# Lucaskabela/UNAST

Hardware: AMD Instinct MI355X
Metric: mel-frames/sec/node (train step, gen+disc) at B=32,T_mel=800; 1/2/4/8-GPU scaling (higher is better)
Workload: dtype bf16x3

## Files before the change

unast_amd/csrc/loss.hip:

```cpp
#include "common.h"

__global__ __launch_bounds__(256) void speech_loss_fwd_kernel(const float* __restrict__ gold, const float* __restrict__ head, int ldh,
                                                              const float* __restrict__ post, const int* __restrict__ lens, int B, int T, int M,
                                                              float eos_weight, double* __restrict__ ws, float* __restrict__ loss) {
    const int rows = B * T;
    const int mq = M >> 2;
    const size_t total = (size_t)rows * mq;
    float a0 = 0.f, a1 = 0.f, a2 = 0.f;
    for (size_t i = (size_t)blockIdx.x * 256 + threadIdx.x; i < total; i += (size_t)gridDim.x * 256) {
        const int r = (int)(i / mq), c = (int)(i - (size_t)r * mq) * 4;
        const int b = r / T, t = r - b * T;
        const int len = lens[b];
        if (t < len) {
            float4 g = *reinterpret_cast<const float4*>(gold + (size_t)r * M + c);
            float4 p = *reinterpret_cast<const float4*>(head + (size_t)r * ldh + c);
            float4 q = *reinterpret_cast<const float4*>(post + (size_t)r * M + c);
            float d;
            d = g.x - p.x; a0 += d * d; d = g.y - p.y; a0 += d * d; d = g.z - p.z; a0 += d * d; d = g.w - p.w; a0 += d * d;
            d = g.x - q.x; a1 += d * d; d = g.y - q.y; a1 += d * d; d = g.z - q.z; a1 += d * d; d = g.w - q.w; a1 += d * d;
        }
        if (c == 0) {
            const float x = head[(size_t)r * ldh + M];
            const float y = (t == len - 1) ? 1.f : 0.f;
            const float lw = 1.f + (eos_weight - 1.f) * y;
// ... 189 lines not shown
                lg[c2][r] = v;
                if (n < V) mx = fmaxf(mx, v);
            }
        mx = fmaxf(mx, __shfl_xor(mx, 16, 64));
        mx = fmaxf(mx, __shfl_xor(mx, 32, 64));
        float se = 0.f, ly = 0.f;
#pragma unroll
        for (int c2 = 0; c2 < 3; ++c2)
#pragma unroll
            for (int r = 0; r < 4; ++r) {
                const int n = 16 * c2 + 4 * g + r;
                if (n < V) se += expf(lg[c2][r] - mx);
                if (n == y) ly = lg[c2][r];
            }
        se += __shfl_xor(se, 16, 64); se += __shfl_xor(se, 32, 64);
        ly += __shfl_xor(ly, 16, 64); ly += __shfl_xor(ly, 32, 64);
        const float wy = (y == pad_idx) ? 0.f : (y == eos_idx ? eos_weight : 1.f);
        const float inv = 1.f / se;
        if (mok) {
#pragma unroll
            for (int c2 = 0; c2 < 3; ++c2) {
                const int n0 = 16 * c2 + 4 * g;
                float4 lo4, dl4;
                float* lp = &lo4.x; float* dp = &dl4.x;
#pragma unroll
                for (int r = 0; r < 4; ++r) {
                    const int n = n0 + r;
                    lp[r] = n < V ? lg[c2][r] : 0.f;
                    dp[r] = n < V ? kg * wy * (expf(lg[c2][r] - mx) * inv - (n == y ? 1.f : 0.f)) : 0.f;
                }
                if (n0 < ldl) {
                    *reinterpret_cast<float4*>(logits + (size_t)m * ldl + n0) = lo4;
                    *reinterpret_cast<float4*>(dlogits + (size_t)m * ldl + n0) = dl4;
                }
            }
            if (g == 0) { a_nll = wy * (logf(se) + mx - ly); a_w = wy; }
        }
    }
    double da = wave_sum_d((double)a_nll), dw = wave_sum_d((double)a_w);
    if (lane == 0 && m0 < rows) { atomicAdd(ws + 0, da); atomicAdd(ws + 1, dw); }
    __syncthreads();
    if (t == 0) {
        __threadfence();
        const unsigned long long arrived = atomicAdd(reinterpret_cast<unsigned long long*>(ws + 3), 1ull) + 1ull;
        if (arrived == gridDim.x) {
            __threadfence();
            const double s0 = atomicAdd(ws + 0, 0.0), s1 = atomicAdd(ws + 1, 0.0);
            loss[0] = (float)(s0 / s1);
            ws[4] = s1;
            ws[0] = 0.0; ws[1] = 0.0; reinterpret_cast<unsigned long long*>(ws)[3] = 0ull;
        }
    }
}

__global__ __launch_bounds__(512) void speech_head_loss_kernel(const float* __restrict__ X, int ldx, const float* __restrict__ W, const float* __restrict__ bias,
                                                               const float* __restrict__ gold, const int* __restrict__ lens, int B, int T, int M,
                                                               float eos_weight, float gscale, float* __restrict__ head, float* __restrict__ d_head, int ldh,
                                                               double* __restrict__ ws) {
    extern __shared__ __attribute__((aligned(16))) unsigned char sdyn[];
    unsigned char* sw0 = sdyn;
    unsigned char* sw1 = sdyn + 96 * 512;
    __shared__ float s_denom;
    const int t = threadIdx.x, lane = t & 63, wave = t >> 6, l15 = lane & 15, g = lane >> 4;
    const int rows = B * T, NO = M + 1;
    for (int i = t; i < 96 * 64; i += 512) {
        const int n = i >> 6, c = (i & 63) * 4;
        float4 v = make_float4(0.f, 0.f, 0.f, 0.f);
        if (n < NO) v = *reinterpret_cast<const float4*>(W + (size_t)n * 256 + c);
        u32x2 hi, lo;
        split4<3>(v, hi, lo);
        *reinterpret_cast<u32x2*>(sw0 + whl_off(n, c)) = hi;
        *reinterpret_cast<u32x2*>(sw1 + whl_off(n, c)) = lo;
    }
    if (t == 0) {
        double sl = 0.0;
        for (int b = 0; b < B; ++b) sl += (double)lens[b];
        s_denom = (float)(sl * (double)M);
    }
    __syncthreads();
    const float km = 2.f * gscale / s_denom, ks = gscale / (float)rows;
    const int m0 = blockIdx.x * 128 + wave * 16;
    const int m = m0 + l15;
    const bool mok = m < rows;
    f32x4 acc[6];
#pragma unroll
    for (int c2 = 0; c2 < 6; ++c2) acc[c2] = (f32x4){0.f, 0.f, 0.f, 0.f};
    float a0 = 0.f, a2 = 0.f;
    if (m0 < rows) {
        const float* xr = X + (size_t)min(m, rows - 1) * ldx;
#pragma unroll
        for (int ks8 = 0; ks8 < 8; ++ks8) {
            const float4 a = *reinterpret_cast<const float4*>(xr + 32 * ks8 + 8 * g);
            const float4 c = *reinterpret_cast<const float4*>(xr + 32 * ks8 + 8 * g + 4);
            u32x2 h0, l0, h1, l1;
            split4<3>(a, h0, l0);
            split4<3>(c, h1, l1);
            const bf16x8_t xh = __builtin_bit_cast(bf16x8_t, (u32x4){h0[0], h0[1], h1[0], h1[1]});
            const bf16x8_t xl = __builtin_bit_cast(bf16x8_t, (u32x4){l0[0], l0[1], l1[0], l1[1]});
#pragma unroll
            for (int c2 = 0; c2 < 6; ++c2) {
                const int off = whl_off(16 * c2 + l15, 32 * ks8 + 8 * g);
                const bf16x8_t wh = *reinterpret_cast<const bf16x8_t*>(sw0 + off);
                const bf16x8_t wlo = *reinterpret_cast<const bf16x8_t*>(sw1 + off);
                acc[c2] = mfma16(wlo, xh, acc[c2]);
                acc[c2] = mfma16(wh, xl, acc[c2]);
                acc[c2] = mfma16(wh, xh, acc[c2]);
            }
        }
        if (mok) {
            const int b = m / T, tt = m - b * T;
            const int len = lens[b];
            const bool live = tt < len;
#pragma unroll
            for (int c2 = 0; c2 < 6; ++c2) {
                const int n0 = 16 * c2 + 4 * g;
                if (n0 >= ldh) continue;
                float4 hv = make_float4(0.f, 0.f, 0.f, 0.f), dv = hv;
                float* hp = &hv.x; float* dp = &dv.x;
                if (n0 < M) {
                    const float4 b4 = *reinterpret_cast<const float4*>(bias + n0);
                    const float bb[4] = {b4.x, b4.y, b4.z, b4.w};
                    float gd[4] = {0.f, 0.f, 0.f, 0.f};
                    if (live) { const float4 g4 = *reinterpret_cast<const float4*>(gold + (size_t)m * M + n0); gd[0] = g4.x; gd[1] = g4.y; gd[2] = g4.z; gd[3] = g4.w; }
#pragma unroll
                    for (int r = 0; r < 4; ++r) {
                        const float p = acc[c2][r] + bb[r];
                        hp[r] = p;
                        if (live) { const float d = p - gd[r]; a0 += d * d; dp[r] = km * d; }
                    }
                } else if (n0 == M) {
                    const float x = acc[c2][0] + bias[M];
                    const float y = (tt == len - 1) ? 1.f : 0.f;
                    const float lw = 1.f + (eos_weight - 1.f) * y;
                    hp[0] = x;
                    a2 += (1.f - y) * x + lw * (log1pf(expf(-fabsf(x))) + fmaxf(-x, 0.f));
                    dp[0] = ks * ((1.f - y) - lw * (1.f - 1.f / (1.f + expf(-x))));
                }
                *reinterpret_cast<float4*>(head + (size_t)m * ldh + n0) = hv;
                *reinterpret_cast<float4*>(d_head + (size_t)m * ldh + n0) = dv;
            }
        }
    }
    __shared__ double red[8][2];
    const double d0 = wave_sum_d((double)a0), d2 = wave_sum_d((double)a2);
    if (lane == 0) { red[wave][0] = d0; red[wave][1] = d2; }
    __syncthreads();
    if (t < 2) {
        double v = 0.0;
        for (int w = 0; w < 8; ++w) v += red[w][t];
        atomicAdd(ws + (t == 0 ? 0 : 2), v);
    }
}

__global__ __launch_bounds__(256) void speech_post_loss_kernel(const float* __restrict__ gold, const float* __restrict__ post, const int* __restrict__ lens,
                                                               int B, int T, int M, float gscale, float* __restrict__ d_post, double* __restrict__ ws,
                                                               float* __restrict__ loss) {
    __shared__ float s_denom;
    if (threadIdx.x == 0) {
        double sl = 0.0;
        for (int b = 0; b < B; ++b) sl += (double)lens[b];
        s_denom = (float)(sl * (double)M);
    }
    __syncthreads();
    const float km = 2.f * gscale / s_denom;
    const int rows = B * T, mq = M >> 2;
    const size_t total = (size_t)rows * mq;
    float a1 = 0.f;
    for (size_t i = (size_t)blockIdx.x * 256 + threadIdx.x; i < total; i += (size_t)gridDim.x * 256) {
        const int r = (int)(i / mq), c = (int)(i - (size_t)r * mq) * 4;
        const int b = r / T, t = r - b * T;
        float4 o = make_float4(0.f, 0.f, 0.f, 0.f);
        if (t < lens[b]) {
            const float4 g = *reinterpret_cast<const float4*>(gold + (size_t)r * M + c);
            const float4 q = *reinterpret_cast<const float4*>(post + (size_t)r * M + c);
            const float dx = q.x - g.x, dy = q.y - g.y, dz = q.z - g.z, dw = q.w - g.w;
            a1 += (dx * dx + dy * dy) + (dz * dz + dw * dw);
            o = make_float4(km * dx, km * dy, km * dz, km * dw);
        }
        *reinterpret_cast<float4*>(d_post + (size_t)r * M + c) = o;
    }
    __shared__ double red[4];
    const double d1 = wave_sum_d((double)a1);
    if ((threadIdx.x & 63) == 0) red[threadIdx.x >> 6] = d1;
    __syncthreads();
    if (threadIdx.x == 0) {
        atomicAdd(ws + 1, (red[0] + red[1]) + (red[2] + red[3]));
        __threadfence();
        const unsigned long long arrived = atomicAdd(reinterpret_cast<unsigned long long*>(ws + 3), 1ull) + 1ull;
        if (arrived == gridDim.x) {
            __threadfence();
            const double s0 = atomicAdd(ws + 0, 0.0), s1 = atomicAdd(ws + 1, 0.0), s2 = atomicAdd(ws + 2, 0.0);
            const double denom = (double)s_denom;
            loss[0] = (float)(s0 / denom + s1 / denom + s2 / ((double)B * T));
            ws[0] = 0.0; ws[1] = 0.0; ws[2] = 0.0; reinterpret_cast<unsigned long long*>(ws)[3] = 0ull;
        }
    }
}

__global__ __launch_bounds__(256) void disc_targets_kernel(const int64_t* __restrict__ perm, int n, int B, int flip, float smoothing, float* __restrict__ out) {
    for (int i = threadIdx.x; i < n; i += 256) {
        float y = 1.f - smoothing;
        if (perm[i] >= B) y = 1.f - y;
        if (flip) y = 1.f - y;
        out[i] = y;
    }
}

__global__ __launch_bounds__(256) void bce_logits_kernel(const float* __restrict__ logits, int ldx, const float* __restrict__ targets, int n,
                                                         const float* __restrict__ gscale, float* __restrict__ loss, float* __restrict__ dlogits, int ldd) {
    __shared__ float red[4];
    float a = 0.f;
    const float g = gscale ? gscale[0] : 0.f;
    for (int i = threadIdx.x; i < n; i += 256) {
        const float y = targets[i];
        const float x = logits[(size_t)i * ldx];
        a += (1.f - y) * x + log1pf(expf(-fabsf(x))) + fmaxf(-x, 0.f);
        if (dlogits) dlogits[(size_t)i * ldd] = g * (1.f / (1.f + expf(-x)) - y) / (float)n;
    }
    a = wave_sum(a);
    if ((threadIdx.x & 63) == 0) red[threadIdx.x >> 6] = a;
    __syncthreads();
    if (threadIdx.x == 0 && loss) loss[0] = ((red[0] + red[1]) + (red[2] + red[3])) / (float)n;
}

static int ls_grid(size_t work, int cap = 1024) {
    size_t b = (work + 255) / 256;
    if (b < 1) b = 1;
    if (b > (size_t)cap) b = cap;
    return (int)b;
}

extern "C" int unast_speech_loss_fwd(const float* gold, const float* head, int ldh, const float* post, const int* lens, int B, int T, int M,
                                     float eos_weight, double* ws , float* loss, hipStream_t stream) {
    UNAST_REQUIRE(gold && head && post && lens && ws && loss, "unast_speech_loss_fwd: null pointer");
    UNAST_REQUIRE(B > 0 && T > 0 && (M & 3) == 0 && ldh > M && (ldh & 3) == 0, "unast_speech_loss_fwd: need M%%4==0 and ldh>M, ldh%%4==0");
    hipLaunchKernelGGL(speech_loss_fwd_kernel, dim3(ls_grid((size_t)B * T * (M / 4), 512)), dim3(256), 0, stream, gold, head, ldh, post, lens, B, T, M,
                       eos_weight, ws, loss);
    return unast_check_launch("unast_speech_loss_fwd");
}

extern "C" int unast_speech_loss_bwd(const float* gold, const float* head, int ldh, const float* post, const int* lens, int B, int T, int M,
                                     float eos_weight, const float* gscale, float* d_head, float* d_post, hipStream_t stream) {
    UNAST_REQUIRE(gold && head && post && lens && gscale && d_head && d_post, "unast_speech_loss_bwd: null pointer");
    UNAST_REQUIRE(B > 0 && T > 0 && (M & 3) == 0 && ldh > M && (ldh & 3) == 0, "unast_speech_loss_bwd: need M%%4==0 and ldh>M, ldh%%4==0");
    hipLaunchKernelGGL(speech_loss_bwd_kernel, dim3(ls_grid((size_t)B * T * (ldh / 4))), dim3(256), 0, stream, gold, head, ldh, post, lens, B, T, M,
                       eos_weight, gscale, d_head, d_post);
    return unast_check_launch("unast_speech_loss_bwd");
}

extern "C" int unast_text_loss_fwd(const float* logits, int ldl, const int64_t* gold, int rows, int V, float eos_weight,
                                   double* ws , float* loss, hipStream_t stream) {
    UNAST_REQUIRE(logits && gold && ws && loss && rows > 0 && V > 0 && ldl >= V, "unast_text_loss_fwd: bad arguments");
    hipLaunchKernelGGL(text_loss_fwd_kernel, dim3(ls_grid(rows)), dim3(256), 0, stream, logits, ldl, gold, rows, V, 2, eos_weight, 0, ws, loss);
    return unast_check_launch("unast_text_loss_fwd");
}

extern "C" int unast_text_loss_bwd(const float* logits, int ldl, const int64_t* gold, int rows, int V, float eos_weight, const double* ws,
                                   const float* gscale, float* dlogits, hipStream_t stream) {
    UNAST_REQUIRE(logits && gold && ws && gscale && dlogits && rows > 0 && V > 0 && ldl >= V, "unast_text_loss_bwd: bad arguments");
    hipLaunchKernelGGL(text_loss_bwd_kernel, dim3(ls_grid(rows)), dim3(256), 0, stream, logits, ldl, gold, rows, V, 2, eos_weight, 0, ws, gscale, dlogits);
    return unast_check_launch("unast_text_loss_bwd");
}

__global__ __launch_bounds__(256) void randperm_kernel(long long* __restrict__ out, int n, uint32_t seed, uint32_t stream) {
    __shared__ uint32_t keys[4096];
    const uint32_t rk = rng_row_key(seed, stream, 0x9E3779B9u);
    for (int i = threadIdx.x; i < n; i += 256) keys[i] = rng_u32(rk, (uint32_t)i);
    __syncthreads();
    for (int i = threadIdx.x; i < n; i += 256) {
        const uint32_t k = keys[i];
        int r = 0;
        for (int j = 0; j < n; ++j) {
            const uint32_t kj = keys[j];
            r += (kj < k || (kj == k && j < i)) ? 1 : 0;
        }
        out[r] = i;
    }
}

extern "C" int unast_randperm(int64_t* out, int n, unsigned int seed, unsigned int stream_id, hipStream_t stream) {
    UNAST_REQUIRE(out && n > 0 && n <= 4096, "unast_randperm: need 0 < n <= 4096 (got %d)", n);
    hipLaunchKernelGGL(randperm_kernel, dim3(1), dim3(256), 0, stream, (long long*)out, n, seed, stream_id);
    return unast_check_launch("unast_randperm");
}

extern "C" int unast_disc_targets(const int64_t* perm, int n, int B, int flip, float smoothing, float* out, hipStream_t stream) {
    UNAST_REQUIRE(perm && out && n > 0, "unast_disc_targets: bad arguments");
    hipLaunchKernelGGL(disc_targets_kernel, dim3(1), dim3(256), 0, stream, perm, n, B, flip, smoothing, out);
    return unast_check_launch("unast_disc_targets");
}

extern "C" int unast_bce_logits(const float* logits, int ldx, const float* targets, int n, const float* gscale, float* loss, float* dlogits,
                                int ldd, hipStream_t stream) {
    UNAST_REQUIRE(logits && targets && n > 0 && ldx >= 1, "unast_bce_logits: bad arguments");
    UNAST_REQUIRE((dlogits == nullptr) || (gscale && ldd >= 1), "unast_bce_logits: dlogits requires gscale and ldd");
    hipLaunchKernelGGL(bce_logits_kernel, dim3(1), dim3(256), 0, stream, logits, ldx, targets, n, gscale, loss, dlogits, ldd);
    return unast_check_launch("unast_bce_logits");
}

__global__ __launch_bounds__(256) void masked_mse_kernel(const float* __restrict__ gold, const float* __restrict__ pred, const float* __restrict__ mask,
                                                         size_t n, double* __restrict__ ws, float* __restrict__ out) {
    double num = 0.0, den = 0.0;
    for (size_t i = (size_t)blockIdx.x * 256 + threadIdx.x; i < n; i += (size_t)gridDim.x * 256) {
        const float d = gold[i] - pred[i], m = mask[i];
        num += (double)(d * d * m);
        den += (double)m;
    }
    num = wave_sum_d(num);
    den = wave_sum_d(den);
    __shared__ double sn[4], sd[4];
    if ((threadIdx.x & 63) == 0) { sn[threadIdx.x >> 6] = num; sd[threadIdx.x >> 6] = den; }
    __syncthreads();
    if (threadIdx.x == 0) {
        atomicAdd(ws + 0, (sn[0] + sn[1]) + (sn[2] + sn[3]));
        atomicAdd(ws + 1, (sd[0] + sd[1]) + (sd[2] + sd[3]));
        __threadfence();
        const unsigned long long arrived = atomicAdd(reinterpret_cast<unsigned long long*>(ws + 2), 1ull) + 1ull;
        if (arrived == gridDim.x) {
            __threadfence();
            const double a = atomicAdd(ws + 0, 0.0), b = atomicAdd(ws + 1, 0.0);
            out[0] = (float)(a / b);
            ws[0] = 0.0; ws[1] = 0.0; reinterpret_cast<unsigned long long*>(ws)[2] = 0ull;
        }
    }
}

extern "C" int unast_masked_mse(const float* gold, const float* pred, const float* mask, int64_t n, double* ws3, float* out, hipStream_t stream) {
    UNAST_REQUIRE(gold && pred && mask && ws3 && out && n > 0, "unast_masked_mse: bad arguments");
    size_t blocks = ((size_t)n + 256 * 8 - 1) / (256 * 8);
    if (blocks > 1024) blocks = 1024;
    hipLaunchKernelGGL(masked_mse_kernel, dim3((unsigned)blocks), dim3(256), 0, stream, gold, pred, mask, (size_t)n, ws3, out);
    return unast_check_launch("unast_masked_mse");
}

__global__ __launch_bounds__(64) void scalar_combine_kernel(const float* __restrict__ a, const float* __restrict__ b, const float* __restrict__ c, float div, float* __restrict__ out) {
    if (threadIdx.x == 0) {
        float s = a[0];
        if (b) s += b[0];
        if (c) s += c[0];
        out[0] = s / div;
    }
}

extern "C" int unast_scalar_combine(const float* a, const float* b, const float* c, float div, float* out, hipStream_t stream) {
    UNAST_REQUIRE(a && out && div != 0.f, "unast_scalar_combine: bad arguments");
    hipLaunchKernelGGL(scalar_combine_kernel, dim3(1), dim3(64), 0, stream, a, b, c, div, out);
    return unast_check_launch("unast_scalar_combine");
}

extern "C" int unast_text_head_loss(const float* X, int ldx, const float* W, const float* bias, const int64_t* gold, int rows, int K, int V,
                                    float eos_weight, float gscale, float* logits, float* dlogits, int ldl, double* ws, float* loss, hipStream_t stream) {
    const int eos_idx = 2, pad_idx = 0;
    UNAST_REQUIRE(X && W && bias && gold && logits && dlogits && ws && loss && rows > 0, "unast_text_head_loss: bad arguments");
    UNAST_REQUIRE(K == 256 && V > 0 && V <= 48 && ldl >= V && ldl <= 48 && (ldl & 3) == 0 && (ldx & 3) == 0, "unast_text_head_loss: built for K = 256, V <= 48, 16-byte row strides (K=%d V=%d ldl=%d)", K, V, ldl);
    UNAST_REQUIRE((((uintptr_t)X | (uintptr_t)W | (uintptr_t)logits | (uintptr_t)dlogits) & 15) == 0, "unast_text_head_loss: operands must be 16-byte aligned");
    hipLaunchKernelGGL(text_head_loss_kernel, dim3((rows + 127) / 128), dim3(512), 0, stream, X, ldx, W, bias, gold, rows, V, eos_idx, eos_weight, pad_idx,
                       gscale, logits, dlogits, ldl, ws, loss);
    return unast_check_launch("unast_text_head_loss");
}

extern "C" int unast_speech_head_loss(const float* X, int ldx, const float* W, const float* bias, const float* gold, const int* lens, int B, int T, int K, int M,
                                      float eos_weight, float gscale, float* head, float* d_head, int ldh, double* ws, hipStream_t stream) {
    UNAST_REQUIRE(X && W && bias && gold && lens && head && d_head && ws && B > 0 && T > 0, "unast_speech_head_loss: bad arguments");
    UNAST_REQUIRE(K == 256 && M > 0 && (M & 3) == 0 && M + 1 <= 96 && ldh >= M + 1 && ldh <= 96 && (ldh & 3) == 0 && (ldx & 3) == 0,
                  "unast_speech_head_loss: built for K = 256, M %% 4 == 0, M + 1 <= 96 (K=%d M=%d ldh=%d)", K, M, ldh);
    UNAST_REQUIRE((((uintptr_t)X | (uintptr_t)W | (uintptr_t)bias | (uintptr_t)gold | (uintptr_t)head | (uintptr_t)d_head) & 15) == 0, "unast_speech_head_loss: operands must be 16-byte aligned");
    static bool attr = [] { return hipFuncSetAttribute((const void*)speech_head_loss_kernel, hipFuncAttributeMaxDynamicSharedMemorySize, 2 * 96 * 512) == hipSuccess; }();
    (void)attr;
    const int rows = B * T;
    hipLaunchKernelGGL(speech_head_loss_kernel, dim3((rows + 127) / 128), dim3(512), 2 * 96 * 512, stream, X, ldx, W, bias, gold, lens, B, T, M, eos_weight, gscale,
                       head, d_head, ldh, ws);
    return unast_check_launch("unast_speech_head_loss");
}

extern "C" int unast_speech_post_loss(const float* gold, const float* post, const int* lens, int B, int T, int M, float gscale, float* d_post, double* ws,
                                      float* loss, hipStream_t stream) {
    UNAST_REQUIRE(gold && post && lens && d_post && ws && loss && B > 0 && T > 0 && M > 0 && (M & 3) == 0, "unast_speech_post_loss: bad arguments");
    hipLaunchKernelGGL(speech_post_loss_kernel, dim3(ls_grid((size_t)B * T * (M / 4))), dim3(256), 0, stream, gold, post, lens, B, T, M, gscale, d_post, ws, loss);
    return unast_check_launch("unast_speech_post_loss");
}

UNAST_DEFINE_RNG_EPOCH_SETTER(loss)
```

unast_amd/csrc/lstm.hip:

```cpp
#include "common.h"
#include "recur.h"

#define LH 64
#define LG (4 * LH)

__device__ __forceinline__ float sigmoidf_(float x) { return __builtin_amdgcn_rcpf(1.f + __expf(-x)); }
__device__ __forceinline__ float tanhf_(float x) { return 2.f * __builtin_amdgcn_rcpf(1.f + __expf(-2.f * x)) - 1.f; }

#define FCH 16
#define BCH 8

#define LOG2E 1.4426950408889634f

__global__ __launch_bounds__(256) void lstm_fwd_kernel(const float* __restrict__ xproj, const float* __restrict__ whh, const float* __restrict__ b_ih,
                                                       const float* __restrict__ b_hh, const int* __restrict__ lens, float* __restrict__ y,
                                                       float* __restrict__ gates, float* __restrict__ cs, float* __restrict__ hprev,
                                                       float* __restrict__ hfinal, int T, int ndir, size_t whh_dir_stride, size_t bias_dir_stride) {
    __shared__ __attribute__((aligned(16))) float h_lds[2][LH];
    const int b = blockIdx.x, dir = blockIdx.y, j = threadIdx.x;
    const int wave = j >> 6, lane = j & 63, q = lane >> 4, c16 = lane & 15;
    const int u = 16 * wave + c16;
    const int row = q * LH + u;
    const int len = lens[b];
    float w[4][16];
// ... 239 lines not shown
    const int t0 = dir ? len - 1 : 0;
    const bool writer = q == 0;
    const __amdgpu_buffer_rsrc_t g_rs = __builtin_amdgcn_make_buffer_rsrc(gates + (size_t)b * T * ndir * WG, 0, (int)((size_t)T * ndir * WG * 4), 0x00020000);
    const uint32_t g_vo = (uint32_t)(dir * WG + row) * 4u;
    int g_so = t0 * ndir * WG * 4;
    const int g_inc = tstep * ndir * WG * 4;
    const float act_m = (q == 2) ? -2.f * LOG2E : -LOG2E, act_s = (q == 2) ? 2.f : 1.f, act_o = (q == 2) ? -1.f : 0.f;
    const size_t st_row0 = ((size_t)b * T + t0) * ndir + dir;
    float* st_p = q == 0 ? cs + st_row0 * WH + u : q == 1 ? y + ((size_t)b * T + t0) * ((size_t)ndir * WH) + dir * WH + u : hprev + st_row0 * WH + u;
    const ptrdiff_t st_inc = (ptrdiff_t)tstep * ndir * WH;
    float xc[FCH], xn[FCH];
    auto load_chunk = [&](int s0, float (&x)[FCH]) {
#pragma unroll
        for (int i = 0; i < FCH; ++i) {
            const int st = min(s0 + i, len - 1);
            x[i] = xp[(size_t)(t0 + st * tstep) * xs];
        }
    };
    load_chunk(0, xn);
    float accn[4] = {0.f, 0.f, 0.f, 0.f};
    for (int s0 = 0; s0 < len; s0 += FCH) {
#pragma unroll
        for (int i = 0; i < FCH; ++i) xc[i] = xn[i] + bias;
        if (s0 + FCH < len) load_chunk(s0 + FCH, xn);
#pragma unroll
        for (int i = 0; i < FCH; ++i) {
            if (s0 + i < len) {
                const float* hl = h_lds[i & 1];
                float hv[WNW];
#pragma unroll
                for (int jw = 1; jw < WNW; ++jw) hv[jw] = hl[hs[jw]];
                float acc[4] = {accn[0] + xc[i], accn[1], accn[2], accn[3]};
#pragma unroll
                for (int jw = 1; jw < WNW; ++jw) dot16<false, false>(w[jw], hv[jw], acc);
                const float pre = (acc[0] + acc[1]) + (acc[2] + acc[3]);
                const float act = __builtin_fmaf(__builtin_amdgcn_rcpf(1.f + __builtin_amdgcn_exp2f(act_m * pre)), act_s, act_o);
                __builtin_amdgcn_raw_buffer_store_b32(__float_as_uint(act), g_rs, g_vo, g_so, 0);
                const float h_before = h;
                float e16, o16, ig, gg, fg, og;
                swap16(act, e16, o16);
                swap32(e16, ig, gg);
                swap32(o16, fg, og);
                c = fg * c + ig * gg;
                h = og * __builtin_fmaf(__builtin_amdgcn_rcpf(1.f + __builtin_amdgcn_exp2f((-2.f * LOG2E) * c)), 2.f, -1.f);
                if (q < 3) *st_p = q == 0 ? c : q == 1 ? h : h_before;
                st_p += st_inc;
                if (writer) h_lds[(i + 1) & 1][u] = h;
                dot16<true, true>(w[0], h, accn);
                g_so += g_inc;
                __syncthreads();
            }
        }
    }
    if (writer) hfinal[(size_t)b * (ndir * WH) + dir * WH + u] = h;
}

__global__ __launch_bounds__(4 * WH) void lstm_bwd128_kernel(const float* __restrict__ dy, const float* __restrict__ dhfinal, const float* __restrict__ whh,
                                                       const float* __restrict__ gates, const float* __restrict__ cs, const int* __restrict__ lens,
                                                       float* __restrict__ dgates, int T, int ndir, size_t whh_dir_stride) {
    __shared__ __attribute__((aligned(16))) float dg_lds[2][WG];
    const int b = blockIdx.x, dir = blockIdx.y, j = threadIdx.x;
    const int len = lens[b];
    const int wave = j >> 6, lane = j & 63, q = lane >> 4, c16 = lane & 15;
    const int k = 16 * wave + c16;
    float wt[WNW][16];
    int src[16];
    RotSrc<0>::fill(c16, src);
    const float* wr = whh + dir * whh_dir_stride + (size_t)(q * WH) * WH + k;
#pragma unroll
    for (int jw = 0; jw < WNW; ++jw)
#pragma unroll
        for (int n = 0; n < 16; ++n) wt[jw][n] = wr[(size_t)(16 * ((wave + jw) & (WNW - 1)) + src[n]) * WH];
    int ds[WNW];
#pragma unroll
    for (int jw = 1; jw < WNW; ++jw) ds[jw] = q * WH + 16 * ((wave + jw) & (WNW - 1)) + c16;
    float dh = 0.f, dc = 0.f;
    if (dhfinal) dh = dhfinal[(size_t)b * (ndir * WH) + dir * WH + k];
    const int tstep = dir ? 1 : -1;
    const int t0 = dir ? 0 : len - 1;
    const __amdgpu_buffer_rsrc_t gl_rs = __builtin_amdgcn_make_buffer_rsrc(const_cast<float*>(gates) + (size_t)b * T * ndir * WG, 0, (int)((size_t)T * ndir * WG * 4), 0x00020000);
    const __amdgpu_buffer_rsrc_t cl_rs = __builtin_amdgcn_make_buffer_rsrc(const_cast<float*>(cs) + (size_t)b * T * ndir * WH, 0, (int)((size_t)T * ndir * WH * 4), 0x00020000);
    const __amdgpu_buffer_rsrc_t yl_rs = __builtin_amdgcn_make_buffer_rsrc(const_cast<float*>(dy ? dy : cs) + (size_t)b * T * ndir * WH, 0, dy ? (int)((size_t)T * ndir * WH * 4) : 0, 0x00020000);
    const int vo_g = (dir * WG + k) * 4, vo_c = (dir * WH + k) * 4;
    auto ldf = [](const __amdgpu_buffer_rsrc_t& rs, int vo, int so) { return __uint_as_float(__builtin_amdgcn_raw_buffer_load_b32(rs, vo, so, 0)); };
    float vn[WBCH][6], cnext;
    const int g_incb = tstep * ndir * WG * 4, c_incb = tstep * ndir * WH * 4;
    auto load_chunk = [&](int r0) {
        int so_g = (t0 + r0 * tstep) * ndir * WG * 4, so_c = (t0 + r0 * tstep) * ndir * WH * 4;
#pragma unroll
        for (int i = 0; i < WBCH; ++i) {
            const int sg = max(so_g, 0), sc = max(so_c, 0);
            vn[i][0] = ldf(gl_rs, vo_g, sg); vn[i][1] = ldf(gl_rs, vo_g + WH * 4, sg); vn[i][2] = ldf(gl_rs, vo_g + 2 * WH * 4, sg); vn[i][3] = ldf(gl_rs, vo_g + 3 * WH * 4, sg);
            vn[i][4] = ldf(cl_rs, vo_c, sc);
            vn[i][5] = ldf(yl_rs, vo_c, sc);
            so_g += g_incb; so_c += c_incb;
        }
        cnext = ldf(cl_rs, vo_c, max(so_c, 0));
    };
    for (int t = max(len, 0); t < T; ++t) dgates[(((size_t)b * T + t) * ndir + dir) * WG + j] = 0.f;
    if (len <= 0) return;
    const __amdgpu_buffer_rsrc_t d_rs = __builtin_amdgcn_make_buffer_rsrc(dgates + (size_t)b * T * ndir * WG, 0, (int)((size_t)T * ndir * WG * 4), 0x00020000);
    const uint32_t d_vo = (uint32_t)(dir * WG + q * WH + k) * 4u;
    int d_so = t0 * ndir * WG * 4;
    const int d_inc = tstep * ndir * WG * 4;
    const bool q0 = q == 0, q1 = q == 1, q2 = q == 2, is_o = q == 3;
    load_chunk(0);
    for (int r0 = 0; r0 < len; r0 += WBCH) {
        float cy[WBCH], cB[WBCH], cf[WBCH], cd[WBCH];
#pragma unroll
        for (int i = 0; i < WBCH; ++i) {
            const float ig = vn[i][0], fg = vn[i][1], gg = vn[i][2], og = vn[i][3];
            const float cafter = i + 1 < WBCH ? vn[i + 1][4] : cnext;
            const float cprev = (r0 + i >= len - 1) ? 0.f : cafter;
            const float tc = tanhf_(vn[i][4]);
            cB[i] = og * (1.f - tc * tc);
            cf[i] = fg;
            cd[i] = vn[i][5];
            const float m1 = q0 ? gg : q1 ? cprev : q2 ? ig : tc;
            const float m2 = q0 ? ig : q1 ? fg : q2 ? gg : og;
            const float ya = m1 * m2, yb = 1.f - m2;
            const float yc = 1.f - m2 * m2;
            cy[i] = q2 ? m1 * yc : ya * yb;
        }
        if (r0 + WBCH < len) load_chunk(r0 + WBCH);
#pragma unroll
        for (int i = 0; i < WBCH; ++i) {
            const int r = r0 + i;
            if (r < len) {
            const float dht = dh + cd[i];
            const float dct = __builtin_fmaf(dht, cB[i], dc);
            dc = dct * cf[i];
            const float mine = (is_o ? dht : dct) * cy[i];
            float* dgw = dg_lds[i & 1];
            dgw[q * WH + k] = mine;
            __builtin_amdgcn_raw_buffer_store_b32(__float_as_uint(mine), d_rs, d_vo, d_so, 0);
            d_so += d_inc;
            float acc[4];
            dot16<true, true>(wt[0], mine, acc);
            __syncthreads();
            float dv[WNW];
#pragma unroll
            for (int jw = 1; jw < WNW; ++jw) dv[jw] = dgw[ds[jw]];
#pragma unroll
            for (int jw = 1; jw < WNW; ++jw) dot16<false, false>(wt[jw], dv[jw], acc);
            float e16, o16, lo, up;
            swap16((acc[0] + acc[1]) + (acc[2] + acc[3]), e16, o16);
            swap32(e16 + o16, lo, up);
            dh = lo + up;
            }
        }
    }
}

__global__ __launch_bounds__(256) void leaky_dropout_kernel(const float* __restrict__ x, const float* __restrict__ dy, float* __restrict__ out, int rows, int D,
                                                            float slope, uint32_t drop_thresh, float drop_scale, uint32_t seed, uint32_t stream) {
    const size_t total = (size_t)rows * D;
    for (size_t i = (size_t)blockIdx.x * 256 + threadIdx.x; i < total; i += (size_t)gridDim.x * 256) {
        const int r = (int)(i / D), c = (int)(i - (size_t)r * D);
        const float xv = x[i];
        float v = dy ? dy[i] * (xv > 0.f ? 1.f : slope) : (xv > 0.f ? xv : xv * slope);
        if (drop_thresh) v = rng_keep(rng_row_key(seed, stream, (uint32_t)r), c, drop_thresh) ? v * drop_scale : 0.f;
        out[i] = v;
    }
}

extern "C" int unast_lstm_fwd(const float* xproj, const float* whh, const float* b_ih, const float* b_hh, const int* lens, float* y, float* gates,
                              float* cs, float* hprev, float* hfinal, int Bd, int T, int ndir, int hidden, int64_t whh_dir_stride,
                              int64_t bias_dir_stride, hipStream_t stream) {
    UNAST_REQUIRE(xproj && whh && b_ih && b_hh && lens && y && gates && cs && hprev && hfinal, "unast_lstm_fwd: null pointer");
    UNAST_REQUIRE(hidden == LH || hidden == WH, "unast_lstm_fwd: this build supports hidden=%d and hidden=%d only (got %d)", LH, WH, hidden);
    UNAST_REQUIRE(Bd > 0 && T > 0 && (ndir == 1 || ndir == 2), "unast_lstm_fwd: bad dims");
    UNAST_REQUIRE((((uintptr_t)whh) & 15) == 0 && (whh_dir_stride & 3) == 0, "unast_lstm_fwd: W_hh must be 16-byte aligned");
    UNAST_REQUIRE((long long)(T + 9) * ndir * 16 * hidden <= 0x7FFFFFFFLL, "unast_lstm_fwd: T=%d is too long for 32-bit offsets into a sequence's slab", T);
    if (hidden == LH)
        hipLaunchKernelGGL(lstm_fwd_kernel, dim3(Bd, ndir), dim3(256), 0, stream, xproj, whh, b_ih, b_hh, lens, y, gates, cs, hprev, hfinal, T, ndir,
                           (size_t)whh_dir_stride, (size_t)bias_dir_stride);
    else
        hipLaunchKernelGGL(lstm_fwd128_kernel, dim3(Bd, ndir), dim3(4 * WH), 0, stream, xproj, whh, b_ih, b_hh, lens, y, gates, cs, hprev, hfinal, T, ndir,
                           (size_t)whh_dir_stride, (size_t)bias_dir_stride);
    return unast_check_launch("unast_lstm_fwd");
}

extern "C" int unast_lstm_bwd(const float* dy, const float* dhfinal, const float* whh, const float* gates, const float* cs, const int* lens,
                              float* dgates, int Bd, int T, int ndir, int hidden, int64_t whh_dir_stride, hipStream_t stream) {
    UNAST_REQUIRE(whh && gates && cs && lens && dgates, "unast_lstm_bwd: null pointer");
    UNAST_REQUIRE(hidden == LH || hidden == WH, "unast_lstm_bwd: this build supports hidden=%d and hidden=%d only (got %d)", LH, WH, hidden);
    UNAST_REQUIRE(Bd > 0 && T > 0 && (ndir == 1 || ndir == 2), "unast_lstm_bwd: bad dims");
    UNAST_REQUIRE((long long)(T + 9) * ndir * 16 * hidden <= 0x7FFFFFFFLL, "unast_lstm_bwd: T=%d is too long for 32-bit offsets into a sequence's slab", T);
    if (hidden == LH)
        hipLaunchKernelGGL(lstm_bwd_kernel, dim3(Bd, ndir), dim3(256), 0, stream, dy, dhfinal, whh, gates, cs, lens, dgates, T, ndir, (size_t)whh_dir_stride);
    else
        hipLaunchKernelGGL(lstm_bwd128_kernel, dim3(Bd, ndir), dim3(4 * WH), 0, stream, dy, dhfinal, whh, gates, cs, lens, dgates, T, ndir,
                           (size_t)whh_dir_stride);
    return unast_check_launch("unast_lstm_bwd");
}

extern "C" int unast_leaky_dropout(const float* x, const float* dy, float* out, int rows, int D, float slope, float drop_p, unsigned int seed,
                                   unsigned int stream_id, hipStream_t stream) {
    UNAST_REQUIRE(x && out && rows > 0 && D > 0, "unast_leaky_dropout: bad arguments");
    size_t blocks = ((size_t)rows * D + 255) / 256;
    if (blocks > 2048) blocks = 2048;
    hipLaunchKernelGGL(leaky_dropout_kernel, dim3((unsigned)blocks), dim3(256), 0, stream, x, dy, out, rows, D, slope, drop_threshold(drop_p),
                       drop_p > 0.f ? 1.f / (1.f - drop_p) : 1.f, seed, stream_id);
    return unast_check_launch("unast_leaky_dropout");
}

UNAST_DEFINE_RNG_EPOCH_SETTER(lstm)
```

unast_amd/csrc/optim.hip:

```cpp
#include "common.h"

__global__ __launch_bounds__(256) void sumsq_kernel(const float* __restrict__ g, size_t n4, size_t n, double* __restrict__ out) {
    float a = 0.f;
    double acc = 0.0;
    int cnt = 0;
    for (size_t i = (size_t)blockIdx.x * 256 + threadIdx.x; i < n4; i += (size_t)gridDim.x * 256) {
        float4 v = reinterpret_cast<const float4*>(g)[i];
        a += (v.x * v.x + v.y * v.y) + (v.z * v.z + v.w * v.w);
        if (++cnt == 64) { acc += (double)a; a = 0.f; cnt = 0; }
    }
    if (blockIdx.x == 0)
        for (size_t i = n4 * 4 + threadIdx.x; i < n; i += 256) a += g[i] * g[i];
    acc += (double)a;
    acc = wave_sum_d(acc);
    if ((threadIdx.x & 63) == 0) atomicAdd(out, acc);
}

__global__ __launch_bounds__(256) void adamw_kernel(float* __restrict__ p, float* __restrict__ g, float* __restrict__ m, float* __restrict__ v,
                                                    size_t n4, size_t n, const double* __restrict__ sumsq, float max_norm, float lr, float b1, float b2,
                                                    float eps, float wd, float bc1, float bc2_sqrt, float* __restrict__ split_out,
                                                    int decoupled, const float* __restrict__ dev_hyper, int zero_grad) {
    if (dev_hyper) { lr = dev_hyper[0]; bc1 = dev_hyper[1]; bc2_sqrt = dev_hyper[2]; }
    float coef = 1.f;
    if (max_norm > 0.f) {
        const float total = (float)sqrt(sumsq[0]);
        coef = fminf(max_norm / (total + 1e-6f), 1.f);
    }
    const float decay = decoupled ? 1.f - lr * wd : 1.f;
    const float l2 = decoupled ? 0.f : wd;
    const float step = lr / bc1;
    auto upd = [&](float& pp, float gg, float& mm, float& vv) {
        gg = gg * coef + l2 * pp;
        pp *= decay;
        mm = mm + (gg - mm) * (1.f - b1);
        vv = vv * b2 + (1.f - b2) * gg * gg;
        const float denom = sqrtf(vv) / bc2_sqrt + eps;
        pp = pp - step * (mm / denom);
    };
    for (size_t i = (size_t)blockIdx.x * 256 + threadIdx.x; i < n4; i += (size_t)gridDim.x * 256) {
        float4 P = reinterpret_cast<float4*>(p)[i], M = reinterpret_cast<float4*>(m)[i], V = reinterpret_cast<float4*>(v)[i];
        const float4 G = reinterpret_cast<const float4*>(g)[i];
        upd(P.x, G.x, M.x, V.x); upd(P.y, G.y, M.y, V.y); upd(P.z, G.z, M.z, V.z); upd(P.w, G.w, M.w, V.w);
        reinterpret_cast<float4*>(p)[i] = P; reinterpret_cast<float4*>(m)[i] = M; reinterpret_cast<float4*>(v)[i] = V;
        if (split_out) reinterpret_cast<uint4*>(split_out)[i] = split_chunk(P);
        if (zero_grad) reinterpret_cast<float4*>(g)[i] = make_float4(0.f, 0.f, 0.f, 0.f);
    }
    if (blockIdx.x == 0)
        for (size_t i = n4 * 4 + threadIdx.x; i < n; i += 256) {
            float pp = p[i], mm = m[i], vv = v[i];
            upd(pp, g[i], mm, vv);
            p[i] = pp; m[i] = mm; v[i] = vv;
            if (zero_grad) g[i] = 0.f;
        }
}

__global__ __launch_bounds__(256) void split_f32_kernel(const float* __restrict__ src, float* __restrict__ dst, size_t n4) {
    for (size_t i = (size_t)blockIdx.x * 256 + threadIdx.x; i < n4; i += (size_t)gridDim.x * 256)
        reinterpret_cast<uint4*>(dst)[i] = split_chunk(reinterpret_cast<const float4*>(src)[i]);
}

extern "C" int unast_sumsq(const float* g, int64_t n, double* out, hipStream_t stream) {
    UNAST_REQUIRE(g && out && n > 0, "unast_sumsq: bad arguments");
    UNAST_REQUIRE((((uintptr_t)g) & 15) == 0, "unast_sumsq: buffer must be 16-byte aligned");
    size_t blocks = ((size_t)n / 4 + 255) / 256;
    if (blocks < 1) blocks = 1;
    if (blocks > 1024) blocks = 1024;
    hipLaunchKernelGGL(sumsq_kernel, dim3((unsigned)blocks), dim3(256), 0, stream, g, (size_t)n / 4, (size_t)n, out);
    return unast_check_launch("unast_sumsq");
}

extern "C" int unast_adamw(float* p, float* g, float* m, float* v, int64_t n, const double* sumsq, float max_norm, float lr,
                           float beta1, float beta2, float eps, float weight_decay, int step, float* split_out, int decoupled,
                           const float* dev_hyper, int zero_grad, hipStream_t stream) {
    UNAST_REQUIRE(p && g && m && v && n > 0 && (step >= 1 || dev_hyper), "unast_adamw: bad arguments");
    if (step < 1) step = 1;
    UNAST_REQUIRE(!(max_norm > 0.f) || sumsq, "unast_adamw: clipping needs the sum-of-squares scalar");
    UNAST_REQUIRE(((((uintptr_t)p) | ((uintptr_t)g) | ((uintptr_t)m) | ((uintptr_t)v)) & 15) == 0, "unast_adamw: buffers must be 16-byte aligned");
    UNAST_REQUIRE(!split_out || ((((uintptr_t)split_out) & 15) == 0 && (n & 3) == 0), "unast_adamw: split_out needs 16-byte alignment and n %% 4 == 0");
    const double bc1 = 1.0 - pow((double)beta1, (double)step);
    const double bc2 = 1.0 - pow((double)beta2, (double)step);
    size_t blocks = ((size_t)n / 4 + 255) / 256;
    if (blocks < 1) blocks = 1;
    if (blocks > 4096) blocks = 4096;
    hipLaunchKernelGGL(adamw_kernel, dim3((unsigned)blocks), dim3(256), 0, stream, p, g, m, v, (size_t)n / 4, (size_t)n, sumsq, max_norm, lr, beta1,
                       beta2, eps, weight_decay, (float)bc1, (float)sqrt(bc2), split_out, decoupled, dev_hyper, zero_grad);
    return unast_check_launch("unast_adamw");
}

struct StepWords { unsigned int w[16]; };
__global__ __launch_bounds__(64) void set_words_kernel(unsigned int* __restrict__ dst, StepWords v, int n) {
    const int i = threadIdx.x;
    if (i < n) dst[i] = v.w[i];
}

extern "C" int unast_set_words(unsigned int* dst, const unsigned int* host_words, int n, hipStream_t stream) {
    UNAST_REQUIRE(dst && host_words && n > 0 && n <= 16, "unast_set_words: need 1..16 words");
    StepWords v;
    for (int i = 0; i < 16; ++i) v.w[i] = i < n ? host_words[i] : 0u;
    hipLaunchKernelGGL(set_words_kernel, dim3(1), dim3(64), 0, stream, dst, v, n);
    return unast_check_launch("unast_set_words");
}

__global__ __launch_bounds__(256) void transpose_split_kernel(const float* __restrict__ src_base, float* __restrict__ dst_base,
                                                              const int* __restrict__ tiles) {
    __shared__ float tile[64][65];
    const int* d = tiles + (size_t)blockIdx.x * 6;
    const int N = d[2], K = d[3], r0 = d[4], c0 = d[5];
    const float* src = src_base + d[0];
    float* dst = dst_base + d[1];
    const int ldT = (N + 3) & ~3;
    const int t = threadIdx.x;
#pragma unroll
    for (int i = 0; i < 4; ++i) {
        const int idx = t + 256 * i, r = idx >> 4, c4 = (idx & 15) * 4;
        float4 v = make_float4(0.f, 0.f, 0.f, 0.f);
        if (r0 + r < N && c0 + c4 < K) v = *reinterpret_cast<const float4*>(src + (size_t)(r0 + r) * K + c0 + c4);
        tile[r][c4] = v.x; tile[r][c4 + 1] = v.y; tile[r][c4 + 2] = v.z; tile[r][c4 + 3] = v.w;
    }
    __syncthreads();
#pragma unroll
    for (int i = 0; i < 4; ++i) {
        const int idx = t + 256 * i, k = idx >> 4, n4 = (idx & 15) * 4;
        if (c0 + k < K && r0 + n4 < ldT)
            *reinterpret_cast<uint4*>(dst + (size_t)(c0 + k) * ldT + r0 + n4) = split_chunk(make_float4(tile[n4][k], tile[n4 + 1][k], tile[n4 + 2][k], tile[n4 + 3][k]));
    }
}

extern "C" int unast_transpose_split(const float* src_base, float* dst_base, const int* tiles_dev, int ntiles, hipStream_t stream) {
    UNAST_REQUIRE(src_base && dst_base && tiles_dev && ntiles > 0, "unast_transpose_split: bad arguments");
    UNAST_REQUIRE(((((uintptr_t)src_base) | ((uintptr_t)dst_base)) & 15) == 0, "unast_transpose_split: bases must be 16-byte aligned");
    hipLaunchKernelGGL(transpose_split_kernel, dim3(ntiles), dim3(256), 0, stream, src_base, dst_base, tiles_dev);
    return unast_check_launch("unast_transpose_split");
}

extern "C" int unast_split_f32(const float* src, float* dst, int64_t n, hipStream_t stream) {
    UNAST_REQUIRE(src && dst && n > 0 && (n & 3) == 0, "unast_split_f32: need n %% 4 == 0 (n=%lld)", (long long)n);
    UNAST_REQUIRE(((((uintptr_t)src) | ((uintptr_t)dst)) & 15) == 0, "unast_split_f32: buffers must be 16-byte aligned");
    size_t blocks = ((size_t)n / 4 + 255) / 256;
    if (blocks > 4096) blocks = 4096;
    hipLaunchKernelGGL(split_f32_kernel, dim3((unsigned)blocks), dim3(256), 0, stream, src, dst, (size_t)n / 4);
    return unast_check_launch("unast_split_f32");
}
```

Measured before the change: 923,700.

## Unroll and widen memory-bound loss, dropout and sumsq kernels

Rewrites three bandwidth-bound elementwise and reduction kernels. The post-mel loss kernel moves to 512 threads, caches sequence lengths in shared memory, issues four loads per thread and uses 32-bit indexing when the size allows. Leaky-ReLU/dropout gets a float4 path with four-way unrolling and keeps a scalar fallback. Gradient sum-of-squares uses eight-way unrolled loads and one atomic per block instead of one per wave. The aim is more memory-level parallelism and fewer atomics, while these kernels are likely a small part of the whole train step.

After: 930,200, median of 6. Within noise of the previous version (+0.7%).

```diff
diff --git a/unast_amd/csrc/loss.hip b/unast_amd/csrc/loss.hip
--- a/unast_amd/csrc/loss.hip
+++ b/unast_amd/csrc/loss.hip
@@ -365,45 +365,86 @@
     }
 }
 
-__global__ __launch_bounds__(256) void speech_post_loss_kernel(const float* __restrict__ gold, const float* __restrict__ post, const int* __restrict__ lens,
-                                                               int B, int T, int M, float gscale, float* __restrict__ d_post, double* __restrict__ ws,
-                                                               float* __restrict__ loss) {
-    __shared__ float s_denom;
-    if (threadIdx.x == 0) {
-        double sl = 0.0;
-        for (int b = 0; b < B; ++b) sl += (double)lens[b];
-        s_denom = (float)(sl * (double)M);
-    }
-    __syncthreads();
-    const float km = 2.f * gscale / s_denom;
-    const int rows = B * T, mq = M >> 2;
-    const size_t total = (size_t)rows * mq;
+constexpr int SPL_THREADS = 512, SPL_BLOCKS = 256, SPL_U = 4, SPL_LENS = 1024;
+template <typename IDX>
+__device__ __forceinline__ float speech_post_loss_body(const float* __restrict__ gold, const float* __restrict__ post, const int* __restrict__ lens,
+                                                       const int* s_lens, int B, int T, int M, float km, float* __restrict__ d_post) {
+    const IDX mq = (IDX)(M >> 2), total = (IDX)B * (IDX)T * mq, stride = (IDX)gridDim.x * SPL_THREADS;
     float a1 = 0.f;
-    for (size_t i = (size_t)blockIdx.x * 256 + threadIdx.x; i < total; i += (size_t)gridDim.x * 256) {
-        const int r = (int)(i / mq), c = (int)(i - (size_t)r * mq) * 4;
-        const int b = r / T, t = r - b * T;
-        float4 o = make_float4(0.f, 0.f, 0.f, 0.f);
-        if (t < lens[b]) {
-            const float4 g = *reinterpret_cast<const float4*>(gold + (size_t)r * M + c);
-            const float4 q = *reinterpret_cast<const float4*>(post + (size_t)r * M + c);
-            const float dx = q.x - g.x, dy = q.y - g.y, dz = q.z - g.z, dw = q.w - g.w;
-            a1 += (dx * dx + dy * dy) + (dz * dz + dw * dw);
-            o = make_float4(km * dx, km * dy, km * dz, km * dw);
-        }
-        *reinterpret_cast<float4*>(d_post + (size_t)r * M + c) = o;
-    }
-    __shared__ double red[4];
+    for (IDX i = (IDX)blockIdx.x * SPL_THREADS + threadIdx.x; i < total; i += SPL_U * stride) {
+        size_t off[SPL_U];
+        bool in[SPL_U], live[SPL_U];
+        float4 g[SPL_U], q[SPL_U];
+#pragma unroll
+        for (int u = 0; u < SPL_U; ++u) {
+            const IDX j = i + (IDX)u * stride;
+            in[u] = j < total;
+            const IDX jj = in[u] ? j : 0;
+            const IDX r = jj / mq;
+            const int c = (int)(jj - r * mq) * 4;
+            const int b = (int)(r / (IDX)T), t = (int)(r - (IDX)b * (IDX)T);
+            off[u] = (size_t)r * M + c;
+            live[u] = in[u] && t < (b < SPL_LENS ? s_lens[b] : lens[b]);
+        }
+#pragma unroll
+        for (int u = 0; u < SPL_U; ++u) {
+            g[u] = q[u] = make_float4(0.f, 0.f, 0.f, 0.f);
+            if (live[u]) {
+                g[u] = *reinterpret_cast<const float4*>(gold + off[u]);
+                q[u] = *reinterpret_cast<const float4*>(post + off[u]);
+            }
+        }
+#pragma unroll
+        for (int u = 0; u < SPL_U; ++u) {
+            float4 o = make_float4(0.f, 0.f, 0.f, 0.f);
+            if (live[u]) {
+                const float dx = q[u].x - g[u].x, dy = q[u].y - g[u].y, dz = q[u].z - g[u].z, dw = q[u].w - g[u].w;
+                a1 += (dx * dx + dy * dy) + (dz * dz + dw * dw);
+                o = make_float4(km * dx, km * dy, km * dz, km * dw);
+            }
+            if (in[u]) *reinterpret_cast<float4*>(d_post + off[u]) = o;
+        }
+    }
+    return a1;
+}
+
+__global__ __launch_bounds__(SPL_THREADS) void speech_post_loss_kernel(const float* __restrict__ gold, const float* __restrict__ post,
+                                                                       const int* __restrict__ lens, int B, int T, int M, float gscale,
+                                                                       float* __restrict__ d_post, double* __restrict__ ws, float* __restrict__ loss) {
+    __shared__ int s_lens[SPL_LENS];
+    __shared__ double red[SPL_THREADS / 64];
+    double sl = 0.0;
+    for (int b = threadIdx.x; b < B; b += SPL_THREADS) {
+        const int l = lens[b];
+        if (b < SPL_LENS) s_lens[b] = l;
+        sl += (double)l;
+    }
+    sl = wave_sum_d(sl);
+    if ((threadIdx.x & 63) == 0) red[threadIdx.x >> 6] = sl;
+    __syncthreads();
+    sl = 0.0;
+#pragma unroll
+    for (int w = 0; w < SPL_THREADS / 64; ++w) sl += red[w];
+    const float denom_f = (float)(sl * (double)M);
+    __syncthreads();
+    const float km = 2.f * gscale / denom_f;
+    const float a1 = (size_t)B * T * (M >> 2) + (size_t)SPL_U * SPL_BLOCKS * SPL_THREADS <= 0xFFFFFFFFull
+                         ? speech_post_loss_body<uint32_t>(gold, post, lens, s_lens, B, T, M, km, d_post)
+                         : speech_post_loss_body<size_t>(gold, post, lens, s_lens, B, T, M, km, d_post);
     const double d1 = wave_sum_d((double)a1);
     if ((threadIdx.x & 63) == 0) red[threadIdx.x >> 6] = d1;
     __syncthreads();
     if (threadIdx.x == 0) {
-        atomicAdd(ws + 1, (red[0] + red[1]) + (red[2] + red[3]));
+        double s = 0.0;
+#pragma unroll
+        for (int w = 0; w < SPL_THREADS / 64; ++w) s += red[w];
+        atomicAdd(ws + 1, s);
         __threadfence();
         const unsigned long long arrived = atomicAdd(reinterpret_cast<unsigned long long*>(ws + 3), 1ull) + 1ull;
         if (arrived == gridDim.x) {
             __threadfence();
             const double s0 = atomicAdd(ws + 0, 0.0), s1 = atomicAdd(ws + 1, 0.0), s2 = atomicAdd(ws + 2, 0.0);
-            const double denom = (double)s_denom;
+            const double denom = (double)denom_f;
             loss[0] = (float)(s0 / denom + s1 / denom + s2 / ((double)B * T));
             ws[0] = 0.0; ws[1] = 0.0; ws[2] = 0.0; reinterpret_cast<unsigned long long*>(ws)[3] = 0ull;
         }
@@ -589,7 +630,9 @@
 extern "C" int unast_speech_post_loss(const float* gold, const float* post, const int* lens, int B, int T, int M, float gscale, float* d_post, double* ws,
                                       float* loss, hipStream_t stream) {
     UNAST_REQUIRE(gold && post && lens && d_post && ws && loss && B > 0 && T > 0 && M > 0 && (M & 3) == 0, "unast_speech_post_loss: bad arguments");
-    hipLaunchKernelGGL(speech_post_loss_kernel, dim3(ls_grid((size_t)B * T * (M / 4))), dim3(256), 0, stream, gold, post, lens, B, T, M, gscale, d_post, ws, loss);
+    const size_t work = (size_t)B * T * (M / 4);
+    hipLaunchKernelGGL(speech_post_loss_kernel, dim3(ls_grid((work + 1) / 2, SPL_BLOCKS)), dim3(SPL_THREADS), 0, stream, gold, post, lens, B, T, M, gscale,
+                       d_post, ws, loss);
     return unast_check_launch("unast_speech_post_loss");
 }
 
diff --git a/unast_amd/csrc/lstm.hip b/unast_amd/csrc/lstm.hip
--- a/unast_amd/csrc/lstm.hip
+++ b/unast_amd/csrc/lstm.hip
@@ -415,8 +415,47 @@
     }
 }
 
+constexpr int LD_U = 4;
 __global__ __launch_bounds__(256) void leaky_dropout_kernel(const float* __restrict__ x, const float* __restrict__ dy, float* __restrict__ out, int rows, int D,
                                                             float slope, uint32_t drop_thresh, float drop_scale, uint32_t seed, uint32_t stream) {
+    const size_t dq = (size_t)(D >> 2), total = (size_t)rows * dq, stride = (size_t)gridDim.x * 256;
+    const bool narrow = total + (size_t)LD_U * stride <= 0xFFFFFFFFull;
+    for (size_t i = (size_t)blockIdx.x * 256 + threadIdx.x; i < total; i += LD_U * stride) {
+        float4 xv[LD_U], dv[LD_U];
+#pragma unroll
+        for (int u = 0; u < LD_U; ++u) {
+            const size_t j = i + u * stride;
+            xv[u] = dv[u] = make_float4(0.f, 0.f, 0.f, 0.f);
+            if (j < total) {
+                xv[u] = reinterpret_cast<const float4*>(x)[j];
+                if (dy) dv[u] = reinterpret_cast<const float4*>(dy)[j];
+            }
+        }
+#pragma unroll
+        for (int u = 0; u < LD_U; ++u) {
+            const size_t j = i + u * stride;
+            if (j >= total) continue;
+            const float xs[4] = {xv[u].x, xv[u].y, xv[u].z, xv[u].w}, ds[4] = {dv[u].x, dv[u].y, dv[u].z, dv[u].w};
+            float v[4];
+#pragma unroll
+            for (int e = 0; e < 4; ++e) v[e] = dy ? ds[e] * (xs[e] > 0.f ? 1.f : slope) : (xs[e] > 0.f ? xs[e] : xs[e] * slope);
+            if (drop_thresh) {
+                const size_t r = narrow ? (size_t)((uint32_t)j / (uint32_t)dq) : j / dq;
+                const uint32_t c = (uint32_t)(j - r * dq) * 4u;
+                const uint32_t rkey = rng_row_key(seed, stream, (uint32_t)r);
+                const uint32_t h0 = rng_pair(rkey, c), h1 = rng_pair(rkey, c + 2u);
+                v[0] = rng_keep_lo(h0, drop_thresh) ? v[0] * drop_scale : 0.f;
+                v[1] = rng_keep_hi(h0, drop_thresh) ? v[1] * drop_scale : 0.f;
+                v[2] = rng_keep_lo(h1, drop_thresh) ? v[2] * drop_scale : 0.f;
+                v[3] = rng_keep_hi(h1, drop_thresh) ? v[3] * drop_scale : 0.f;
+            }
+            reinterpret_cast<float4*>(out)[j] = make_float4(v[0], v[1], v[2], v[3]);
+        }
+    }
+}
+
+__global__ __launch_bounds__(256) void leaky_dropout_scalar_kernel(const float* __restrict__ x, const float* __restrict__ dy, float* __restrict__ out, int rows, int D,
+                                                                   float slope, uint32_t drop_thresh, float drop_scale, uint32_t seed, uint32_t stream) {
     const size_t total = (size_t)rows * D;
     for (size_t i = (size_t)blockIdx.x * 256 + threadIdx.x; i < total; i += (size_t)gridDim.x * 256) {
         const int r = (int)(i / D), c = (int)(i - (size_t)r * D);
@@ -461,10 +500,15 @@
 extern "C" int unast_leaky_dropout(const float* x, const float* dy, float* out, int rows, int D, float slope, float drop_p, unsigned int seed,
                                    unsigned int stream_id, hipStream_t stream) {
     UNAST_REQUIRE(x && out && rows > 0 && D > 0, "unast_leaky_dropout: bad arguments");
-    size_t blocks = ((size_t)rows * D + 255) / 256;
+    const bool vec = (D & 3) == 0 && ((((uintptr_t)x) | ((uintptr_t)dy) | ((uintptr_t)out)) & 15) == 0;
+    size_t blocks = ((size_t)rows * (vec ? D / 4 : D) + 255) / 256;
     if (blocks > 2048) blocks = 2048;
-    hipLaunchKernelGGL(leaky_dropout_kernel, dim3((unsigned)blocks), dim3(256), 0, stream, x, dy, out, rows, D, slope, drop_threshold(drop_p),
-                       drop_p > 0.f ? 1.f / (1.f - drop_p) : 1.f, seed, stream_id);
+    if (vec)
+        hipLaunchKernelGGL(leaky_dropout_kernel, dim3((unsigned)blocks), dim3(256), 0, stream, x, dy, out, rows, D, slope, drop_threshold(drop_p),
+                           drop_p > 0.f ? 1.f / (1.f - drop_p) : 1.f, seed, stream_id);
+    else
+        hipLaunchKernelGGL(leaky_dropout_scalar_kernel, dim3((unsigned)blocks), dim3(256), 0, stream, x, dy, out, rows, D, slope, drop_threshold(drop_p),
+                           drop_p > 0.f ? 1.f / (1.f - drop_p) : 1.f, seed, stream_id);
     return unast_check_launch("unast_leaky_dropout");
 }
 
diff --git a/unast_amd/csrc/optim.hip b/unast_amd/csrc/optim.hip
--- a/unast_amd/csrc/optim.hip
+++ b/unast_amd/csrc/optim.hip
@@ -1,19 +1,37 @@
 #include "common.h"
 
-__global__ __launch_bounds__(256) void sumsq_kernel(const float* __restrict__ g, size_t n4, size_t n, double* __restrict__ out) {
-    float a = 0.f;
+constexpr int SUMSQ_THREADS = 512, SUMSQ_BLOCKS = 256, SUMSQ_U = 8;
+__global__ __launch_bounds__(SUMSQ_THREADS) void sumsq_kernel(const float* __restrict__ g, size_t n4, size_t n, double* __restrict__ out) {
+    __shared__ double red[SUMSQ_THREADS / 64];
+    const float4* __restrict__ g4 = reinterpret_cast<const float4*>(g);
+    const size_t stride = (size_t)gridDim.x * SUMSQ_THREADS;
     double acc = 0.0;
-    int cnt = 0;
-    for (size_t i = (size_t)blockIdx.x * 256 + threadIdx.x; i < n4; i += (size_t)gridDim.x * 256) {
-        float4 v = reinterpret_cast<const float4*>(g)[i];
-        a += (v.x * v.x + v.y * v.y) + (v.z * v.z + v.w * v.w);
-        if (++cnt == 64) { acc += (double)a; a = 0.f; cnt = 0; }
+    for (size_t i = (size_t)blockIdx.x * SUMSQ_THREADS + threadIdx.x; i < n4; i += SUMSQ_U * stride) {
+        float4 v[SUMSQ_U];
+#pragma unroll
+        for (int u = 0; u < SUMSQ_U; ++u) {
+            const size_t j = i + u * stride;
+            v[u] = j < n4 ? g4[j] : make_float4(0.f, 0.f, 0.f, 0.f);
+        }
+        float a = 0.f;
+#pragma unroll
+        for (int u = 0; u < SUMSQ_U; ++u) a += (v[u].x * v[u].x + v[u].y * v[u].y) + (v[u].z * v[u].z + v[u].w * v[u].w);
+        acc += (double)a;
     }
-    if (blockIdx.x == 0)
-        for (size_t i = n4 * 4 + threadIdx.x; i < n; i += 256) a += g[i] * g[i];
-    acc += (double)a;
+    if (blockIdx.x == 0) {
+        float a = 0.f;
+        for (size_t i = n4 * 4 + threadIdx.x; i < n; i += SUMSQ_THREADS) a += g[i] * g[i];
+        acc += (double)a;
+    }
     acc = wave_sum_d(acc);
-    if ((threadIdx.x & 63) == 0) atomicAdd(out, acc);
+    if ((threadIdx.x & 63) == 0) red[threadIdx.x >> 6] = acc;
+    __syncthreads();
+    if (threadIdx.x == 0) {
+        double s = 0.0;
+#pragma unroll
+        for (int w = 0; w < SUMSQ_THREADS / 64; ++w) s += red[w];
+        atomicAdd(out, s);
+    }
 }
 
 __global__ __launch_bounds__(256) void adamw_kernel(float* __restrict__ p, float* __restrict__ g, float* __restrict__ m, float* __restrict__ v,
@@ -62,10 +80,10 @@
 extern "C" int unast_sumsq(const float* g, int64_t n, double* out, hipStream_t stream) {
     UNAST_REQUIRE(g && out && n > 0, "unast_sumsq: bad arguments");
     UNAST_REQUIRE((((uintptr_t)g) & 15) == 0, "unast_sumsq: buffer must be 16-byte aligned");
-    size_t blocks = ((size_t)n / 4 + 255) / 256;
+    size_t blocks = ((size_t)n / 4 + SUMSQ_THREADS - 1) / SUMSQ_THREADS;
     if (blocks < 1) blocks = 1;
-    if (blocks > 1024) blocks = 1024;
-    hipLaunchKernelGGL(sumsq_kernel, dim3((unsigned)blocks), dim3(256), 0, stream, g, (size_t)n / 4, (size_t)n, out);
+    if (blocks > SUMSQ_BLOCKS) blocks = SUMSQ_BLOCKS;
+    hipLaunchKernelGGL(sumsq_kernel, dim3((unsigned)blocks), dim3(SUMSQ_THREADS), 0, stream, g, (size_t)n / 4, (size_t)n, out);
     return unast_check_launch("unast_sumsq");
 }
 
```
